# williamyang98/FM-Radio

Hardware: AMD Instinct MI355X
Metric: IQ MSamples/sec demodulated to stereo+RDS per GPU; channels @ real-time (higher is better)
Workload: dtype f32 (tolerance mode: FIR operands split into 2 x bf16 on the matrix cores, 3 products per tap, fp32 accumulate; everything else fp32)

## Files before the change

fm-radio_amd/csrc/fmd_kernels_bp.inc:

```
struct ExtractGeomB {
    static constexpr int TA = 256, WN = 4 * TA + 188, WNP = 1216;
    static constexpr int NBW = (WNP + 8 * (WNP >> 5)) / 2;
    static constexpr int KS = 8;
    static constexpr int EDGE = 124;
    __device__ static __forceinline__ int pad(int i) { return i + 8 * (i >> 5); }
    static_assert(WNP % 32 == 0 && WNP >= 64 * 15 + 32 * KS, "reach of the operands");
    static_assert(WN % 4 == 0 && WN / 4 - 256 <= 64 && WNP / 4 - 256 <= 64, "four quads per lane and one more for lanes 0 .. 47 stage the window");
};
static constexpr int kBpTabU4 = kBpTL * 2 / 16, kBpTabSlotU4 = kBpSlotTabs * kBpTabU4;
static_assert(kBpTL * 2 % 256 == 128 && kBpTL >= kBpPadL + 4 + 32 * ExtractGeomB::KS + 8 && kBpPadL >= 32 + 4 * 14 + 8 && kBpPadL % 8 == 0, "tap table geometry");

__device__ __forceinline__ float oct_sum_f32(float v) {
    {
        const int up = __builtin_amdgcn_update_dpp(0, __float_as_int(v), 0x104, 0xf, 0x5, true);
        v += __int_as_float(__builtin_amdgcn_update_dpp(up, __float_as_int(v), 0x114, 0xf, 0xA, false));
    }
    v += dpp0<0x4E>(v);
    v += dpp0<0xB1>(v);
    return v;
}

template <int SPW>
__global__ __launch_bounds__(256, 4) void k_extract_bp(Dims d, int nt, const float* __restrict__ fo_pl, const float4* __restrict__ pll_poly,
                                                        const uint4* __restrict__ bp_tab, const int2* __restrict__ aud_idx, const uint4* __restrict__ rds_tab,
                                                        const uint4* __restrict__ bp_edge, const float* __restrict__ mixctl, float* __restrict__ state,
                                                        float* __restrict__ audio, float2* __restrict__ rds, float* __restrict__ lmr_est,
                                                        float* __restrict__ lpr_out, float* __restrict__ lmr_out, int keep_taps,
                                                        const float* __restrict__ lmr_est_prev, int field_cur, int field_prev, float* __restrict__ rds_pow) {
    using G = ExtractGeomB;
    constexpr int TA = G::TA;
    __shared__ __attribute__((aligned(256))) uint16_t tabs[(kBpSlotTabs + kBpRdsTabs) * kBpTL];
    __shared__ __attribute__((aligned(16))) uint32_t win[4][2 * G::NBW];
    __shared__ float2 s_old[SPW][SPW == 1 ? 32 : 31];
    __shared__ float off_s[SPW];
    float* wf32 = reinterpret_cast<float*>(win[3]);
    static_assert(sizeof(tabs) + sizeof(win) + sizeof(s_old) + sizeof(off_s) <= 40960, "four workgroups per CU");

    const bool no_edge = (nt & 0x10000) != 0;
    nt &= 0xffff;
    const int tiles = d.n_audio / TA, per_wg = 4 * nt, groups = (tiles + per_wg - 1) / per_wg;
    const int c = SPW * (blockIdx.x / groups), tile_first = (blockIdx.x % groups) * per_wg;
    const bool two = SPW == 2 && c + 1 < d.C;
    const int tid = threadIdx.x;
    __builtin_assume(tid >= 0 && tid < 256);
    const int lane = tid & (kWave - 1), wv = __builtin_amdgcn_readfirstlane(tid >> 6);
    const int n = d.n_fm_out;
    const float* fo_c0 = fo_pl + (size_t)c * (kFoPad + n) + kFoPad;
    const float4* po_c0 = pll_poly + (size_t)c * (1 + n / kSpan) + 1;
    const float off_prev0 = st(state, field_prev, d.C, c), off_prev1 = two ? st(state, field_prev, d.C, c + 1) : 0.0f;
    float off_cur0 = lmr_est_prev ? 0.0f : st(state, field_cur, d.C, c), off_cur1 = (lmr_est_prev || !two) ? 0.0f : st(state, field_cur, d.C, c + 1);
    const bool edge = tile_first == 0 && !no_edge;
#ifdef FMD_X_PROBE
    const bool xp_on = (blockIdx.x % 61) == 0;
    unsigned long long xp_t = __builtin_readcyclecounter();
    const unsigned long long xp_c0 = xp_t, xp_w0 = wall_clock64();
    if (xp_on && threadIdx.x == 0) atomicAdd(&g_x_probe[7], (unsigned long long)nt);
#endif

    float ev[kLmrInlineMax / kWave];
    const bool est_wave = wv == 0 || (wv == 1 && two);
    if (lmr_est_prev && est_wave) {
#pragma unroll
        for (int k = 0; k < kLmrInlineMax / kWave; k++) ev[k] = (lane + kWave * k < d.n_est) ? lmr_est_prev[(size_t)(c + wv) * d.n_est + lane + kWave * k] : 0.0f;
    }
    uint4 em[kBpEdgeU4];
    float4 qe, qe1;
    {
        const int2 slot = aud_idx[c];
        if (edge) {
            if (tid < 48) qe = *reinterpret_cast<const float4*>(fo_c0 - 188 + 4 * tid);
            if (SPW == 2 && two && tid < 48) qe1 = *reinterpret_cast<const float4*>(fo_c0 + (kFoPad + n) - 188 + 4 * tid);
            if (tid < kBpEdgeRows) {
                const uint4* ep = bp_edge + ((size_t)slot.y * kBpEdgeRows + tid) * kBpEdgeU4;
#pragma unroll
                for (int k = 0; k < kBpEdgeU4; k++) em[k] = ep[k];
            }
        }
        constexpr int NU4 = (kBpSlotTabs + kBpRdsTabs) * kBpTabU4;
#pragma unroll
        for (int r = 0; r < (NU4 + 255) / 256; r++) {
            const int j = tid + 256 * r;
            if (j < NU4) {
                const int blk = j / (4 * kBpTabU4), within = j % (4 * kBpTabU4);
                const uint4* src = blk == 0 ? bp_tab + (size_t)slot.x * kBpTabSlotU4 + within
                                 : (blk < 3 ? bp_tab + (size_t)slot.y * kBpTabSlotU4 + blk * 4 * kBpTabU4 + within : rds_tab + (blk - 3) * 4 * kBpTabU4 + within);
                reinterpret_cast<uint4*>(tabs)[j] = *src;
            }
        }
    }
    const int mode0 = (int)mixctl[2 * c], mode1 = two ? (int)mixctl[2 * c + 2] : 0;
    const float kmix0 = mixctl[2 * c + 1], kmix1 = two ? mixctl[2 * c + 3] : 0.0f;
    if (lmr_est_prev && est_wave) {
        float part = 0.0f;
#pragma unroll
        for (int k = 0; k < kLmrInlineMax / kWave; k++) part += ev[k];
        float nxt = fmaf(wave_sum_f32(part) * __builtin_amdgcn_rcpf((float)d.n_est), 0.1f, wv ? off_prev1 : off_prev0);
        const float two_pi = bits_f32(kTwoPiBits);
        nxt = (nxt >= two_pi) ? nxt - two_pi : ((nxt <= -two_pi) ? nxt + two_pi : nxt);
        if (lane == 0) { off_s[wv] = nxt; if (tile_first == 0) st(state, field_cur, d.C, c + wv) = nxt; }
    }
#pragma unroll
    for (int sx = 0; sx < SPW; sx++) {
      if (edge && (sx == 0 || two)) {
        if (sx) __syncthreads();
        if (tid < 48) *reinterpret_cast<float4*>(wf32 + 4 * tid) = sx ? qe1 : qe;
        __syncthreads();
        if (tid < kBpEdgeRows) {
            const float* wp = wf32 + 24 * (tid & 7);
            float ar = 0.0f, ai = 0.0f;
            typedef _Float16 h2_t __attribute__((ext_vector_type(2)));
#pragma unroll
            for (int k = 0; k < kBpEdgeU4; k++) {
                const float4 w4 = *reinterpret_cast<const float4*>(wp + 4 * k);
                const uint32_t ew[4] = {em[k].x, em[k].y, em[k].z, em[k].w};
                const float ws[4] = {w4.x, w4.y, w4.z, w4.w};
#pragma unroll
                for (int u = 0; u < 4; u++) {
                    const h2_t e = __builtin_bit_cast(h2_t, ew[u]);
                    ar = fmaf((float)e[0], ws[u], ar); ai = fmaf((float)e[1], ws[u], ai);
                }
            }
            ar = oct_sum_f32(ar); ai = oct_sum_f32(ai);
            if ((tid & 7) == 0) s_old[sx][tid >> 3] = make_float2(ar, ai);
        }
      }
    }
    __syncthreads();
    if (lmr_est_prev) { off_cur0 = off_s[0]; if (SPW == 2 && two) off_cur1 = off_s[1]; }
    X_STAMP(1);

    uint32_t* fh = win[wv];
    uint32_t* fl = fh + G::NBW;
    float4 qw[5];
    const int tiles_wg = two ? 2 * tiles : tiles;
    auto wload = [&](int tix) {
        const int sx = (SPW == 2 && tix >= tiles) ? 1 : 0, tile = tix - sx * tiles;
        const float* wsrc = fo_c0 + (size_t)sx * (kFoPad + n) + (4 * tile * TA - 188);
#pragma unroll
        for (int r = 0; r < 4; r++) qw[r] = ld_mid(reinterpret_cast<const float4*>(wsrc + 4 * (lane + 64 * r)));
        const int q4 = 256 + lane;
        qw[4] = ld_mid(reinterpret_cast<const float4*>(wsrc + 4 * (q4 < G::WN / 4 ? q4 : G::WN / 4 - 1)));
    };
    if (tile_first + wv < tiles_wg) wload(tile_first + wv);
    for (int it = 0; it < nt; it++) {
        const int tix = tile_first + 4 * it + wv;
        if (tix >= tiles_wg) break;
        const int sx = (SPW == 2 && tix >= tiles) ? 1 : 0, tile = tix - sx * tiles, i0 = tile * TA;
        const int cc = c + sx;
        const float4* po_c = po_c0 + (size_t)sx * (1 + n / kSpan);
        const float off_prev = sx ? off_prev1 : off_prev0, off_cur = sx ? off_cur1 : off_cur0, kmix = sx ? kmix1 : kmix0;
        const int mode = sx ? mode1 : mode0;
        int ln = lane;
        asm volatile("" : "+v"(ln));
        __builtin_assume(ln >= 0 && ln < 64);
        const int lrow = ln & 15, lq = ln >> 4;
        const int m0 = i0 + 16 * lrow + 4 * lq, r0 = (i0 >> 1) + 8 * lrow + 2 * lq;
        const int tc2a = 8 * m0 - 121, tc2r = 16 * r0 - 113;

        {
            auto put = [&](int q, const float4& v) {
                uint32_t h0, l0, h1, l1, h2, l2, h3, l3;
                split_bf16(v.x, h0, l0); split_bf16(v.y, h1, l1); split_bf16(v.z, h2, l2); split_bf16(v.w, h3, l3);
                const int w = G::pad(4 * q) >> 1;
                *reinterpret_cast<uint2*>(fh + w) = make_uint2(pack_hi16(h0, h1), pack_hi16(h2, h3));
                *reinterpret_cast<uint2*>(fl + w) = make_uint2(pack_hi16(l0, l1), pack_hi16(l2, l3));
            };
#pragma unroll
            for (int r = 0; r < 4; r++) put(ln + 64 * r, qw[r]);
            if (ln < G::WNP / 4 - 256) put(256 + ln, (256 + ln >= G::WN / 4) ? make_float4(0.f, 0.f, 0.f, 0.f) : qw[4]);
        }
        const float4 pva = po_c[tc2a >> 8], pvr = po_c[tc2r >> 8];
        asm volatile("s_waitcnt lgkmcnt(0)" ::: "memory");
        __builtin_amdgcn_wave_barrier();
        X_STAMP(0);

        f32x4 acc[4] = {kZero4, kZero4, kZero4, kZero4}, s1 = kZero4;
        {
            const int wb = G::pad(64 * lrow + 8 * lq) >> 1;
            const uint16_t* ta = tabs + (lrow & 1) * kBpTL + kBpPadL + 8 * lq - 4 * (lrow & ~1);
            const uint16_t* t3 = tabs + (12 + (lrow & 1)) * kBpTL + kBpPadL + 8 * lq - 8 * (lrow >> 1);
            auto ld = [](const void* p) { return __builtin_bit_cast(bf16x8, *reinterpret_cast<const uint4*>(p)); };
#pragma unroll
            for (int sK = 0; sK < G::KS; sK++) {
                const bf16x8 bh = ld(fh + wb + 20 * sK), bl = ld(fl + wb + 20 * sK);
                bf16x8 ah[4], al[4];
                ah[0] = ld(ta - 32 + 32 * sK);               al[0] = ld(ta - 32 + 2 * kBpTL + 32 * sK);
                ah[1] = ld(ta + 4 * kBpTL + 32 * sK);        al[1] = ld(ta + 6 * kBpTL + 32 * sK);
                ah[2] = ld(ta + 8 * kBpTL + 32 * sK);        al[2] = ld(ta + 10 * kBpTL + 32 * sK);
                ah[3] = ld(t3 + 32 * sK);                    al[3] = ld(t3 + 2 * kBpTL + 32 * sK);
                const bf16x8 a1 = ld(t3 + 4 * kBpTL + 32 * sK);
#pragma unroll
                for (int f = 0; f < 4; f++) acc[f] = __builtin_amdgcn_mfma_f32_16x16x32_bf16(ah[f], bh, acc[f], 0, 0, 0);
#pragma unroll
                for (int f = 0; f < 4; f++) acc[f] = __builtin_amdgcn_mfma_f32_16x16x32_bf16(al[f], bh, acc[f], 0, 0, 0);
#pragma unroll
                for (int f = 0; f < 4; f++) acc[f] = __builtin_amdgcn_mfma_f32_16x16x32_bf16(ah[f], bl, acc[f], 0, 0, 0);
                s1 = __builtin_amdgcn_mfma_f32_16x16x32_bf16(a1, bh, s1, 0, 0, 0);
#ifndef FMD_BP_SB
#define FMD_BP_SB 1
#endif
                if ((sK % FMD_BP_SB) == FMD_BP_SB - 1) __builtin_amdgcn_sched_barrier(0);
            }
        }
        asm volatile("" ::: "memory");
        X_STAMP(2);
        if (it + 1 < nt && tix + 4 < tiles_wg) wload(tix + 4);

        {
            const float uc0 = 0.5f * (float)(tc2a & 255);
            float dc = 0.0f, ds = 0.0f;
            if (tile == 0) {
                const float dph = off_prev - off_cur;
                dc = fast_cos_turns(dph) - 1.0f; ds = fast_sin_turns(dph);
            }
            float lmr_v[4], lre_v[4], lpr_v[4], au[8];
#pragma unroll
            for (int i = 0; i < 4; i++) {
                const int m = m0 + i;
                const float uc = uc0 + 4.0f * (float)i;
                const float p = fmaf(fmaf(fmaf(pva.w, uc, pva.z), uc, pva.y), uc, pva.x);
                const float nom = (float)((-38 * (4 * (m + 1) - 127)) & 127) * (1.0f / 128.0f);
                float2 sv = make_float2(acc[1][i], acc[2][i]);
                if (tile == 0 && 16 * lrow + 4 * lq + i < 31) {
                    const float2 so = s_old[sx][16 * lrow + 4 * lq + i];
                    sv.x += fmaf(dc, so.x, -(ds * so.y)); sv.y += fmaf(dc, so.y, ds * so.x);
                }
                const float ph = fmaf(2.0f, p, nom) + off_cur;
                const float cs = fast_cos_turns(ph), sn = fast_sin_turns(ph);
                const float lmr_re = fmaf(sv.x, cs, -(sv.y * sn)), lmr = fmaf(sv.x, sn, sv.y * cs);
                const float lpr = acc[0][i];
                float l, r;
                if (mode == FMD_AUDIO_STEREO) { l = fmaf(lmr, kmix, lpr); r = fmaf(-lmr, kmix, lpr); }
                else if (mode == FMD_AUDIO_LMR) { l = lmr; r = lmr; }
                else { l = lpr; r = lpr; }
                au[2 * i] = l + l; au[2 * i + 1] = r + r;
                lmr_v[i] = lmr; lre_v[i] = lmr_re; lpr_v[i] = lpr;
            }
            float4* ap = reinterpret_cast<float4*>(audio + 2 * ((size_t)cc * d.n_audio + m0));
            st_stream(ap, make_float4(au[0], au[1], au[2], au[3])); st_stream(ap + 1, make_float4(au[4], au[5], au[6], au[7]));
            if (keep_taps) {
                *reinterpret_cast<float4*>(lpr_out + (size_t)cc * d.n_audio + m0) = make_float4(lpr_v[0], lpr_v[1], lpr_v[2], lpr_v[3]);
                *reinterpret_cast<float4*>(lmr_out + (size_t)cc * d.n_audio + m0) = make_float4(lmr_v[0], lmr_v[1], lmr_v[2], lmr_v[3]);
            }
            {
                const int k10 = (10 - m0 % 10) % 10;
                if (k10 < 4) {
                    const float a = k10 == 0 ? lmr_v[0] : (k10 == 1 ? lmr_v[1] : (k10 == 2 ? lmr_v[2] : lmr_v[3]));
                    const float b = k10 == 0 ? lre_v[0] : (k10 == 1 ? lre_v[1] : (k10 == 2 ? lre_v[2] : lre_v[3]));
                    const float pe = fast_atan2f(a, b);
                    const float half_pi = bits_f32(kHalfPiBits);
                    lmr_est[(size_t)cc * d.n_est + (m0 + k10) / 10] = (pe > 0.0f) ? (half_pi - pe) : (-half_pi - pe);
                }
            }
            {
                const float ur0 = 0.5f * (float)(tc2r & 255);
                float y[4], pw[2];
#pragma unroll
                for (int j = 0; j < 2; j++) {
                    const int ri = r0 + j;
                    const float ur = ur0 + 8.0f * (float)j;
                    const float pr = fmaf(fmaf(fmaf(pvr.w, ur, pvr.z), ur, pvr.y), ur, pvr.x);
                    const float dpr = fmaf(fmaf(3.0f * pvr.w, ur, 2.0f * pvr.z), ur, pvr.y);
                    const float nomr = (float)((-57 * (8 * (ri + 1) - 127)) & 127) * (1.0f / 128.0f);
                    const float eps = bits_f32(kTwoPiBits) * 3.0f * dpr;
                    const float xr = fmaf(-eps, s1[2 * j + 1], acc[3][2 * j]), xi = fmaf(eps, s1[2 * j], acc[3][2 * j + 1]);
                    const float phr = fmaf(3.0f, pr, nomr);
                    const float cr = fast_cos_turns(phr), sr = fast_sin_turns(phr);
                    y[2 * j] = fmaf(xr, cr, -(xi * sr)); y[2 * j + 1] = fmaf(xr, sr, xi * cr);
                    pw[j] = wave_sum_f32(fmaf(y[2 * j], y[2 * j], y[2 * j + 1] * y[2 * j + 1]));
                }
                *reinterpret_cast<float4*>(rds + (size_t)cc * d.n_rds + r0) = make_float4(y[0], y[1], y[2], y[3]);
                if (ln == 0) *reinterpret_cast<float2*>(rds_pow + ((size_t)cc * tiles + tile) * 2) = make_float2(pw[0], pw[1]);
            }
        }
        X_STAMP(3);
        X_STAMP(4);
    }
#ifdef FMD_X_PROBE
    if (xp_on && (threadIdx.x & 63) == 0 && (threadIdx.x >> 6) == 0) { atomicAdd(&g_x_probe2[7], __builtin_readcyclecounter() - xp_c0); atomicAdd(&g_x_probe2[15], wall_clock64() - xp_w0); }
#endif
}
```

fm-radio_amd/csrc/fmd_tables.cpp:

```cpp
#include "fmd_tables.h"

#include <cmath>
#include <complex>
#include <cstring>
#include <vector>

#include "fmd_design.h"
#include "fmd_math.h"
#include "fmdemod_debug.h"

namespace fmd {

static uint16_t bf16_rne(float x) {
    uint32_t u; std::memcpy(&u, &x, 4);
    u += 0x7fffu + ((u >> 16) & 1u);
    return (uint16_t)(u >> 16);
}
static float bf16_to_f32(uint16_t h) { const uint32_t u = (uint32_t)h << 16; float x; std::memcpy(&x, &u, 4); return x; }
static void toeplitz_image(const float* taps, int n_taps, int stride, int ksteps, uint16_t* img, int shift = 0) {
    for (int sK = 0; sK < ksteps; sK++)
        for (int l = 0; l < 64; l++)
            for (int i = 0; i < 8; i++) {
                const int t = 32 * sK + 8 * (l / 16) + i, idx = t - shift - stride * (l % 16);
                const float v = (idx >= 0 && idx < n_taps) ? taps[idx] : 0.0f;
                const uint16_t hi = bf16_rne(v), lo = bf16_rne(v - bf16_to_f32(hi));
                img[(((size_t)sK * 2 + 0) * 64 + l) * 8 + i] = hi;
                img[(((size_t)sK * 2 + 1) * 64 + l) * 8 + i] = lo;
            }
}

static void bandpass_taps(const float* h, const float* b_hil, int H, float* g_re, float* g_im) {
    double re[kBpTaps] = {0.0}, im[kBpTaps] = {0.0};
    const double two_pi = 6.283185307179586476925;
    for (int tau = 0; tau < 128; tau++) {
        const int k = (H * 19 * tau) % 128;
        const double cr = std::cos(two_pi * k / 128.0), ci = -std::sin(two_pi * k / 128.0), hv = h[tau];
        re[tau + 32] += hv * cr; im[tau + 32] += hv * ci;
        for (int n = 0; n < 65; n++) {
            const double b = b_hil[n];
            if (b == 0.0) continue;
            re[tau + n] += hv * (-ci) * b;
            im[tau + n] += hv * cr * b;
        }
    }
    for (int u = 0; u < kBpTaps; u++) { g_re[u] = (float)re[u]; g_im[u] = (float)im[u]; }
}
static void bp_tap_table(const float* taps, int n_taps, int move, uint16_t* hi, uint16_t* lo) {
    for (int i = 0; i < kBpTL; i++) { hi[i] = 0; if (lo) lo[i] = 0; }
    for (int i = 0; i < n_taps; i++) {
        const uint16_t h = bf16_rne(taps[i]);
        hi[kBpPadL + move + i] = h;
        if (lo) lo[kBpPadL + move + i] = bf16_rne(taps[i] - bf16_to_f32(h));
    }
}
static void bp_family_block(const float* taps, int n_taps, uint16_t* dst) {
    bp_tap_table(taps, n_taps, 0, dst, dst + 2 * kBpTL);
    bp_tap_table(taps, n_taps, 4, dst + kBpTL, dst + 3 * kBpTL);
}
void bp_slot_tap_tables(const float* taps, const float* b_hil, uint16_t* dst) {
    bp_family_block(taps, 128, dst);
    float gr[kBpTaps], gi[kBpTaps];
    bandpass_taps(taps, b_hil, 2, gr, gi);
    bp_family_block(gr, kBpTaps, dst + 4 * kBpTL);
    bp_family_block(gi, kBpTaps, dst + 8 * kBpTL);
}
void bp_rds_tap_tables(const float* b_rds, const float* b_hil, uint16_t* dst) {
    float gr[kBpTaps], gi[kBpTaps], h1[128];
    bandpass_taps(b_rds, b_hil, 3, gr, gi);
    bp_tap_table(gr, kBpTaps, 4, dst, dst + 2 * kBpTL);
    bp_tap_table(gi, kBpTaps, 4, dst + kBpTL, dst + 3 * kBpTL);
    for (int i = 0; i < 128; i++) h1[i] = (float)(((double)i - 63.5) * (double)b_rds[i]);
    bandpass_taps(h1, b_hil, 3, gr, gi);
    bp_tap_table(gr, kBpTaps, 4, dst + 4 * kBpTL, nullptr);
    bp_tap_table(gi, kBpTaps, 4, dst + 5 * kBpTL, nullptr);
}

static uint16_t f32_to_f16_rne(float x) {
    uint32_t u; std::memcpy(&u, &x, 4);
    const uint32_t sign = (u >> 16) & 0x8000u;
    const int e = (int)((u >> 23) & 0xffu) - 127 + 15;
    uint32_t m = u & 0x7fffffu;
    if (e >= 31) return (uint16_t)(sign | 0x7c00u);
    if (e <= 0) {
        if (e < -10) return (uint16_t)sign;
        m |= 0x800000u;
        const int sh = 14 - e;
        const uint32_t r = m >> sh, rem = m & ((1u << sh) - 1u), half = 1u << (sh - 1);
        return (uint16_t)(sign | (r + ((rem > half || (rem == half && (r & 1u))) ? 1u : 0u)));
    }
    const uint32_t r = ((uint32_t)e << 10) | (m >> 13), rem = m & 0x1fffu;
    return (uint16_t)(sign | (r + ((rem > 0x1000u || (rem == 0x1000u && (r & 1u))) ? 1u : 0u)));
}
void bp_edge_matrix(const float* taps, const float* b_hil, uint16_t* dst) {
    constexpr int NM = kBpEdgeRows / 8, NC = kBpEdgeU4 * 4;
    static_assert(8 * NC == kBpTaps, "eight lanes share an output's taps");
    std::memset(dst, 0, sizeof(uint16_t) * kBpEdgeHalves);
    for (int m = 0; m < NM; m++) {
        float ht[128], gr[kBpTaps], gi[kBpTaps];
        for (int i = 0; i < 128; i++) ht[i] = i < 124 - 4 * m ? taps[i] : 0.0f;
        bandpass_taps(ht, b_hil, 2, gr, gi);
        for (int u = 0; u < kBpTaps; u++) {
            const int idx = u - 4 * m;
            if (idx < 0 || idx >= kBpTaps) continue;
            uint16_t* e = dst + (((size_t)m * 8 + u / NC) * NC + u % NC) * 2;
            e[0] = f32_to_f16_rne(gr[idx]); e[1] = f32_to_f16_rne(gi[idx]);
        }
    }
}

void design_pilot_fast(const fmd_coeffs& k, PilotFastTab* t) {
    const double a0 = k.pilot_a[0], a1 = k.pilot_a[1];
    struct M2 { double a, b, c, d; };
    auto mul = [](const M2& x, const M2& y) { return M2{x.a * y.a + x.b * y.c, x.a * y.b + x.b * y.d, x.c * y.a + x.d * y.c, x.c * y.b + x.d * y.d}; };
    const M2 A{a1, a0, 1.0, 0.0};
    M2 P = A;
    for (int i = 0; i < kPilotSeg; i++) { t->h1[i] = (float)P.a; t->h2[i] = (float)P.b; if (i + 1 < kPilotSeg) P = mul(A, P); }
    M2 S = P;
    for (int s = 0; s < 4; s++) { t->m[s][0] = (float)S.a; t->m[s][1] = (float)S.b; t->m[s][2] = (float)S.c; t->m[s][3] = (float)S.d; S = mul(S, S); }
    M2 L{1.0, 0.0, 0.0, 1.0};
    for (int l = 0; l <= 32; l++) { t->mlane[l][0] = (float)L.a; t->mlane[l][1] = (float)L.b; t->mlane[l][2] = (float)L.c; t->mlane[l][3] = (float)L.d; L = mul(P, L); }
    t->k = k.pilot_b[0]; t->a0 = k.pilot_a[0]; t->a1 = k.pilot_a[1];
}

static void span_rows(const fmd_coeffs& k, std::vector<double> (&rows)[kSpanRows]) {
    constexpr int L = kSpan, NV = 5 + L;
    const double b0 = k.pll_lpf_b[0], b1 = k.pll_lpf_b[1], a0 = k.pll_lpf_a[0];
    const float Ts32 = 1.0f / 128000.0f;
    const double Ts = (double)Ts32, ktsi = (double)(0.1f * Ts32), two_pi = 6.283185307179586476925;
    using Vec = std::vector<double>;
    auto unit = [&](int i) { Vec v(NV, 0.0); v[(size_t)i] = 1.0; return v; };
    Vec lpf = unit(0), I = unit(1), e1 = unit(2), e2 = unit(3), dev(NV, 0.0), g0;
    for (int n = 0; n < L; n++) {
        Vec g(NV), e(NV);
        for (int i = 0; i < NV; i++) {
            lpf[i] = b0 * e2[i] + b1 * e1[i] + a0 * lpf[i];
            I[i] += ktsi * e1[i];
            g[i] = -100.0 * (0.01 * lpf[i] + I[i]);
        }
        if (n == 0) g0 = g;
        for (int i = 0; i < NV; i++) dev[i] += Ts * (g[i] - g0[i]);
        dev[4] -= Ts;
        for (int i = 0; i < NV; i++) e[i] = two_pi * dev[i];
        e[5 + n] += two_pi;
        if (n == kSpanN1) rows[2] = dev;
        if (n == kSpanN2) rows[3] = dev;
        if (n == L - 1) { rows[0] = lpf; rows[1] = I; rows[4] = dev; }
        e2 = e1; e1 = e;
    }
}

static void span_cubic_inverse(float (&minv)[3][4]) {
    constexpr int L = kSpan;
    const double x[3] = {(double)kSpanN1, (double)kSpanN2, (double)(L - 1)};
    double A[3][3], inv[3][3];
    for (int i = 0; i < 3; i++) { A[i][0] = x[i]; A[i][1] = x[i] * x[i]; A[i][2] = x[i] * x[i] * x[i]; }
    const double det = A[0][0] * (A[1][1] * A[2][2] - A[1][2] * A[2][1]) - A[0][1] * (A[1][0] * A[2][2] - A[1][2] * A[2][0]) + A[0][2] * (A[1][0] * A[2][1] - A[1][1] * A[2][0]);
    for (int i = 0; i < 3; i++)
        for (int j = 0; j < 3; j++) {
            const int i1 = (i + 1) % 3, i2 = (i + 2) % 3, j1 = (j + 1) % 3, j2 = (j + 2) % 3;
            inv[j][i] = (A[i1][j1] * A[i2][j2] - A[i1][j2] * A[i2][j1]) / det;
        }
    for (int i = 0; i < 3; i++) { for (int j = 0; j < 3; j++) minv[i][j] = (float)inv[i][j]; minv[i][3] = 0.0f; }
}

void design_pll_span(const fmd_coeffs& k, PllSpanTab* t) {
    constexpr int L = kSpan;
    const float Ts32 = 1.0f / 128000.0f;
    const double Ts = (double)Ts32, two_pi = 6.283185307179586476925;
    std::vector<double> rows[kSpanRows];
    span_rows(k, rows);
    std::memset(t, 0, sizeof(*t));
    for (int r = 0; r < kSpanRows; r++) {
        for (int n = 0; n < L; n++) t->w[r][n] = (float)rows[r][(size_t)(5 + n)];
        for (int i = 0; i < 5; i++) t->s[r][i] = (float)rows[r][(size_t)i];
    }
    span_cubic_inverse(t->minv);
    const double w0 = two_pi * 19000.0 / 128000.0;
    double hr = 0.0, hi = 0.0;
    for (int i = 0; i < 65; i++) { hr += k.b_hilbert[i] * std::cos(w0 * i); hi += k.b_hilbert[i] * std::sin(w0 * i); }
    t->quad = (float)(std::sqrt(hr * hr + hi * hi) / (2.0 * std::sin(w0)));
    t->kappa = (float)(-19000.0 * Ts + 19.0 / 128.0);
    for (int i = 0; i < 32; i++) t->hil[i] = k.b_hilbert[2 * i + 1];
}

void design_pll_sparse(const fmd_coeffs& k, PllSparseTab* t) {
    using cd = std::complex<double>;
    constexpr int L = kSpan, D = kSparseDec, KP = kSparsePts;
    const double two_pi = 6.283185307179586476925, w0 = two_pi * 19.0 / 128.0;
    const float Ts32 = 1.0f / 128000.0f;
    std::memset(t, 0, sizeof(*t));
    const double r = std::sqrt(-(double)k.pilot_a[0]), wp = std::acos((double)k.pilot_a[1] / (2.0 * r));
    const cd rho = std::polar(r, wp - w0);
    cd W[2 * D];
    for (int q = -8; q < 24; q++) {
        cd acc = 0.0;
        for (int i = 0; i < D; i++) if (std::abs(q - i) <= 8) acc += std::pow(rho, i);
        W[q + 8] = acc / 17.0;
    }
    cd wcd[2 * D];
    for (int tt = 0; tt < 2 * D; tt++) {
        wcd[tt] = W[(23 - tt) + 8] * std::polar(1.0, -w0 * (double)(tt - 46));
        t->wre[tt] = (float)wcd[tt].real(); t->wim[tt] = (float)wcd[tt].imag();
    }
    const cd rho16 = std::pow(rho, D);
    for (int kk = 0; kk < KP; kk++) {
        const cd ro = std::polar(1.0, -w0 * (double)(D * kk)), ca = std::pow(rho16, kk + 1);
        t->rot[kk][0] = (float)ro.real(); t->rot[kk][1] = (float)ro.imag();
        t->carry[kk][0] = (float)ca.real(); t->carry[kk][1] = (float)ca.imag();
        t->nk1[kk] = (float)(D * kk + 10);
    }
    double nbar = 0.0, s2 = 0.0;
    for (int kk = 0; kk < KP; kk++) nbar += (double)(D * kk + 9) / KP;
    for (int kk = 0; kk < KP; kk++) { const double c = (double)(D * kk + 9) - nbar; t->ck[kk] = (float)c; s2 += c * c; }
    for (int s_ = 0; s_ < 3; s_++) { const cd p = std::pow(rho16, 1 << s_); t->scan[s_][0] = (float)p.real(); t->scan[s_][1] = (float)p.imag(); }
    const cd cA = cd(0.0, -1.0) * ((double)k.pilot_b[0] / std::sin(wp)) * std::polar(1.0, wp);
    double phi0 = std::arg(cA) / two_pi - 19.0 * 33.0 / 128.0;
    phi0 -= std::nearbyint(phi0);
    t->phi0 = (float)phi0; t->inv_s2 = (float)(1.0 / s2); t->nbar = (float)nbar;
    t->kappa = (float)(-19000.0 * (double)Ts32 + 19.0 / 128.0);
    double hr = 0.0, hi = 0.0;
    for (int i = 0; i < 65; i++) { hr += k.b_hilbert[i] * std::cos(w0 * i); hi += k.b_hilbert[i] * std::sin(w0 * i); }
    const double g2 = hr * hr + hi * hi;
    t->pw_scale = (float)(std::norm(cA) * (1.0 + g2) * 0.5 * (double)D);
    cd wdc = 0.0;
    for (int q = 0; q < 2 * D; q++) wdc += W[q];
    const cd kap2 = -std::polar(1.0, -2.0 * wp) / (wdc * (1.0 - std::polar(r, -(wp + w0))));
    t->kap2[0] = (float)kap2.real(); t->kap2[1] = (float)kap2.imag();
    std::vector<double> rows[kSpanRows];
    span_rows(k, rows);
    {
        float mi[3][4];
        span_cubic_inverse(mi);
        const std::vector<double> d1 = rows[2], d2 = rows[3], d3 = rows[4];
        for (int i = 0; i < 3; i++)
            for (size_t j = 0; j < d1.size(); j++) rows[2 + i][j] = (double)mi[i][0] * d1[j] + (double)mi[i][1] * d2[j] + (double)mi[i][2] * d3[j];
    }
    for (int rr = 0; rr < kSpanRows; rr++) {
        double ws = 0.0, wm = 0.0, suf = 0.0;
        for (int n = L - 1; n >= 0; n--) {
            const double w = rows[rr][(size_t)(5 + n)];
            ws += w; wm += w * ((double)n - nbar); suf += w;
            t->sw[rr][n] = (float)suf;
        }
        t->wsum[rr] = (float)ws; t->wmom[rr] = (float)wm;
        for (int i = 0; i < 5; i++) t->s[rr][i] = (float)rows[rr][(size_t)i];
    }
}

void design_wrap_tie(uint32_t* bits2048) {
    std::memset(bits2048, 0, sizeof(uint32_t) * 2048);
    const float pi = fmd::bits_f32(fmd::kPiBits), two_pi = fmd::bits_f32(fmd::kTwoPiBits);
    for (int yr = 0; yr < 256; yr++)
        for (int xr = 0; xr < 256; xr++) {
            const float x = (float)xr - 127.0f, y = (float)yr - 127.0f;
            if (x == 0.0f && y == 0.0f) continue;
            float dl = fmd::fmd_atan2f_full(0.0f - y, 0.0f - x) - fmd::fmd_atan2f_full(y, x);
            if (dl >= pi) dl = dl - two_pi;
            else if (dl <= -pi) dl = dl + two_pi;
            const unsigned key = ((unsigned)yr << 8) | (unsigned)xr;
            if (dl > 0.0f) bits2048[key >> 5] |= 1u << (key & 31u);
        }
}

void design_front_mfma(const fmd_coeffs& k, int m, std::vector<uint16_t>& img) {
    const int ks_pre = m > 1 ? predecim_ksteps(m) : 0;
    img.assign(((size_t)kFrontImgU4 + (size_t)ks_pre * kImgKStepU4) * 8, 0);
    toeplitz_image(k.b_fm_out, 64, 2, 3, img.data());
    toeplitz_image(k.b_hilbert, 65, 1, 3, img.data() + (size_t)kFrontImgU4 / 2 * 8);
    if (m > 1) toeplitz_image(k.b_fm_in, 64, m, ks_pre, img.data() + (size_t)kFrontImgU4 * 8, predecim_shift(m));
}

}

using namespace fmd;

int fmd_design_pll_span(int fs_baseband, float* w, float* s, float* minv, float* misc2) {
    if (!w || !s || !minv || !misc2) return FMD_ERR_ARG;
    if (fs_baseband != 256000 && fs_baseband != 1024000 && fs_baseband != 2048000) return FMD_ERR_ARG;
    fmd_controls def;
    fmd_default_controls(&def);
    fmd_coeffs k{};
    design_all(&k, fs_baseband, &def);
    PllSpanTab t;
    design_pll_span(k, &t);
    std::memcpy(w, t.w, sizeof(t.w)); std::memcpy(s, t.s, sizeof(t.s)); std::memcpy(minv, t.minv, sizeof(t.minv));
    misc2[0] = t.quad; misc2[1] = t.kappa;
    return FMD_OK;
}

int fmd_design_pll_sparse(int fs_baseband, float* taps, float* cplx, float* rows, float* sw, float* misc8) {
    if (!taps || !cplx || !rows || !sw || !misc8) return FMD_ERR_ARG;
    if (fs_baseband != 256000 && fs_baseband != 1024000 && fs_baseband != 2048000) return FMD_ERR_ARG;
    fmd_controls def;
    fmd_default_controls(&def);
    fmd_coeffs k{};
    design_all(&k, fs_baseband, &def);
    PllSparseTab t;
    design_pll_sparse(k, &t);
    std::memcpy(taps, t.wre, sizeof(t.wre)); std::memcpy(taps + 2 * kSparseDec, t.wim, sizeof(t.wim));
    std::memcpy(cplx, t.rot, sizeof(t.rot)); std::memcpy(cplx + 16, t.scan, sizeof(t.scan)); std::memcpy(cplx + 22, t.carry, sizeof(t.carry));
    std::memcpy(rows, t.wsum, sizeof(t.wsum)); std::memcpy(rows + 8, t.wmom, sizeof(t.wmom));
    std::memcpy(sw, t.sw, sizeof(t.sw));
    const float m[8] = {t.phi0, t.inv_s2, t.nbar, t.kappa, t.pw_scale, t.kap2[0], t.kap2[1], 0.f};
    std::memcpy(misc8, m, sizeof(m));
    return FMD_OK;
}

int fmd_design_wrap_tie(uint32_t* bits2048) {
    if (!bits2048) return FMD_ERR_ARG;
    design_wrap_tie(bits2048);
    return FMD_OK;
}

int fmd_design_extract_bp(int fs_baseband, int cutoff_hz, float* g2, float* g3) {
    if (!g2 || !g3) return FMD_ERR_ARG;
    fmd_controls c;
    fmd_default_controls(&c);
    c.lmr_cutoff_hz = cutoff_hz;
    fmd_coeffs k{};
    design_all(&k, fs_baseband, &c);
    bandpass_taps(k.b_lmr, k.b_hilbert, 2, g2, g2 + kBpTaps);
    bandpass_taps(k.b_rds, k.b_hilbert, 3, g3, g3 + kBpTaps);
    return FMD_OK;
}
```

fm-radio_amd/csrc/fmd_tables.h:

```cpp
#pragma once

#include <stddef.h>
#include <stdint.h>
#include <vector>

#include "fmdemod.h"

namespace fmd {

static constexpr int kPilotSeg = 8;
struct PilotFastTab {
    float h1[kPilotSeg], h2[kPilotSeg];
    float m[4][4];
    float mlane[33][4];
    float k, a0, a1;
};

static constexpr int kSpan = 128;
static constexpr int kSpanN1 = 41, kSpanN2 = 84;
static constexpr int kSpanRows = 5;
struct PllSpanTab {
    float w[kSpanRows][kSpan];
    float s[kSpanRows][8];
    float minv[3][4];
    float quad;
    float kappa;
    float pad[2];
    float hil[32];
};
static constexpr int kSparsePts = 8, kSparseDec = kSpan / kSparsePts;
static constexpr float kPllWarmSamples = 8192.0f;
struct PllSparseTab {
    float wre[2 * kSparseDec], wim[2 * kSparseDec];
    float rot[kSparsePts][2];
    float scan[3][2];
    float carry[kSparsePts][2];
    float ck[kSparsePts];
    float nk1[kSparsePts];
    float phi0;
    float inv_s2, nbar, kappa, pw_scale;
    float kap2[2], pad_;
    float wsum[8], wmom[8];
    float s[kSpanRows][8];
    float sw[kSpanRows][kSpan + 4];
    uint32_t wrap_tie[2048];
};
static constexpr int kImgKStepU4 = 2 * 64;
static constexpr int kFrontImgU4 = 2 * 3 * kImgKStepU4;
constexpr int predecim_shift(int m) { return 8 - m; }
constexpr int predecim_ksteps(int m) { return (64 + predecim_shift(m) + 15 * m + 31) / 32; }
static constexpr int kFoPad = 192;

static constexpr int kBpTaps = 192;
static constexpr int kBpPadL = 96, kBpTL = 448;
static constexpr int kBpSlotTabs = 12, kBpRdsTabs = 6;
static constexpr size_t kBpTabSlotU16 = (size_t)kBpSlotTabs * kBpTL, kBpRdsTabU16 = (size_t)kBpRdsTabs * kBpTL;
static constexpr int kBpEdgeRows = 31 * 8, kBpEdgeU4 = 6;
static constexpr size_t kBpEdgeHalves = (size_t)kBpEdgeRows * kBpEdgeU4 * 8;

void design_pilot_fast(const fmd_coeffs& k, PilotFastTab* t);
void design_pll_span(const fmd_coeffs& k, PllSpanTab* t);
void design_pll_sparse(const fmd_coeffs& k, PllSparseTab* t);
void design_wrap_tie(uint32_t* bits2048);
void design_front_mfma(const fmd_coeffs& k, int m, std::vector<uint16_t>& img);
void bp_slot_tap_tables(const float* taps, const float* b_hil, uint16_t* dst);
void bp_rds_tap_tables(const float* b_rds, const float* b_hil, uint16_t* dst);
void bp_edge_matrix(const float* taps, const float* b_hil, uint16_t* dst);

}
```

Baseline: 264,900.

## Give each wave consecutive tiles, slide the LDS window, skip zero-tap L+R MFMAs

Each wave now handles a contiguous run of tiles rather than interleaving with stride 4. That lets it keep the overlapping tail of the previous split-bf16 window in LDS, slide it forward, and convert only the new quads instead of reloading and re-splitting the whole window. The L+R filter family skips the first and last K-steps, whose 128-tap table holds only zeros, removing three MFMAs per skipped step. This trades the prior cross-wave load balancing and coalescing pattern for less global traffic and conversion work, plus an extra LDS copy with an explicit wait.

Measured after the change: 261,100. 0.986x the previous value.

```diff
diff --git a/fm-radio_amd/csrc/fmd_kernels_bp.inc b/fm-radio_amd/csrc/fmd_kernels_bp.inc
--- a/fm-radio_amd/csrc/fmd_kernels_bp.inc
+++ b/fm-radio_amd/csrc/fmd_kernels_bp.inc
@@ -3,10 +3,18 @@
     static constexpr int NBW = (WNP + 8 * (WNP >> 5)) / 2;
     static constexpr int KS = 8;
     static constexpr int EDGE = 124;
+    static constexpr int ROW = 4;
+    static constexpr int LPR_SHIFT = 32;
+    static constexpr int SLIDE_G0 = 4 * TA / 32, SLIDE_GROUPS = (WNP - 4 * TA) / 32, NEW_Q0 = (WN - 4 * TA) / 4;
     __device__ static __forceinline__ int pad(int i) { return i + 8 * (i >> 5); }
+    static constexpr bool lpr_step(int s) { return 32 * s + 31 - LPR_SHIFT >= 0 && 32 * s - LPR_SHIFT - ROW * 15 < kBpLprTaps; }
+    static_assert((4 * TA) % 32 == 0 && SLIDE_G0 + SLIDE_GROUPS == WNP / 32 && 4 * SLIDE_GROUPS * 2 <= 64 && WN / 4 - NEW_Q0 == 256 && WNP / 4 - WN / 4 == 1,
+                  "slide: whole padded groups, a 16-byte move per lane, four new quads per lane, one quad of zeros behind the window");
     static_assert(WNP % 32 == 0 && WNP >= 64 * 15 + 32 * KS, "reach of the operands");
     static_assert(WN % 4 == 0 && WN / 4 - 256 <= 64 && WNP / 4 - 256 <= 64, "four quads per lane and one more for lanes 0 .. 47 stage the window");
 };
+static_assert(!ExtractGeomB::lpr_step(0) && !ExtractGeomB::lpr_step(ExtractGeomB::KS - 1) && ExtractGeomB::lpr_step(1) && ExtractGeomB::lpr_step(ExtractGeomB::KS - 2),
+              "L+R: K-steps 0 and KS - 1 multiply zero taps only (and are left out), the others do not");
 static constexpr int kBpTabU4 = kBpTL * 2 / 16, kBpTabSlotU4 = kBpSlotTabs * kBpTabU4;
 static_assert(kBpTL * 2 % 256 == 128 && kBpTL >= kBpPadL + 4 + 32 * ExtractGeomB::KS + 8 && kBpPadL >= 32 + 4 * 14 + 8 && kBpPadL % 8 == 0, "tap table geometry");
 
@@ -57,6 +65,19 @@
     if (xp_on && threadIdx.x == 0) atomicAdd(&g_x_probe[7], (unsigned long long)nt);
 #endif
 
+    float4 qw[5];
+    const int tiles_wg = two ? 2 * tiles : tiles, tix0 = tile_first + wv * nt;
+    auto wload = [&](int tix, bool slide) {
+        const int sx = (SPW == 2 && tix >= tiles) ? 1 : 0, tile = tix - sx * tiles;
+        const float* wsrc = fo_c0 + (size_t)sx * (kFoPad + n) + (4 * tile * TA - 188) + (slide ? 4 * G::NEW_Q0 : 0);
+#pragma unroll
+        for (int r = 0; r < 4; r++) qw[r] = ld_mid(reinterpret_cast<const float4*>(wsrc + 4 * (lane + 64 * r)));
+        if (!slide) {
+            const int q4 = 256 + lane;
+            qw[4] = ld_mid(reinterpret_cast<const float4*>(wsrc + 4 * (q4 < G::WN / 4 ? q4 : G::WN / 4 - 1)));
+        }
+    };
+
     float ev[kLmrInlineMax / kWave];
     const bool est_wave = wv == 0 || (wv == 1 && two);
     if (lmr_est_prev && est_wave) {
@@ -88,6 +109,7 @@
             }
         }
     }
+    if (tix0 < tiles_wg) wload(tix0, false);
     const int mode0 = (int)mixctl[2 * c], mode1 = two ? (int)mixctl[2 * c + 2] : 0;
     const float kmix0 = mixctl[2 * c + 1], kmix1 = two ? mixctl[2 * c + 3] : 0.0f;
     if (lmr_est_prev && est_wave) {
@@ -131,21 +153,11 @@
 
     uint32_t* fh = win[wv];
     uint32_t* fl = fh + G::NBW;
-    float4 qw[5];
-    const int tiles_wg = two ? 2 * tiles : tiles;
-    auto wload = [&](int tix) {
-        const int sx = (SPW == 2 && tix >= tiles) ? 1 : 0, tile = tix - sx * tiles;
-        const float* wsrc = fo_c0 + (size_t)sx * (kFoPad + n) + (4 * tile * TA - 188);
-#pragma unroll
-        for (int r = 0; r < 4; r++) qw[r] = ld_mid(reinterpret_cast<const float4*>(wsrc + 4 * (lane + 64 * r)));
-        const int q4 = 256 + lane;
-        qw[4] = ld_mid(reinterpret_cast<const float4*>(wsrc + 4 * (q4 < G::WN / 4 ? q4 : G::WN / 4 - 1)));
-    };
-    if (tile_first + wv < tiles_wg) wload(tile_first + wv);
     for (int it = 0; it < nt; it++) {
-        const int tix = tile_first + 4 * it + wv;
+        const int tix = tix0 + it;
         if (tix >= tiles_wg) break;
         const int sx = (SPW == 2 && tix >= tiles) ? 1 : 0, tile = tix - sx * tiles, i0 = tile * TA;
+        const bool slide = it > 0 && tile != 0;
         const int cc = c + sx;
         const float4* po_c = po_c0 + (size_t)sx * (1 + n / kSpan);
         const float off_prev = sx ? off_prev1 : off_prev0, off_cur = sx ? off_cur1 : off_cur0, kmix = sx ? kmix1 : kmix0;
@@ -165,9 +177,20 @@
                 *reinterpret_cast<uint2*>(fh + w) = make_uint2(pack_hi16(h0, h1), pack_hi16(h2, h3));
                 *reinterpret_cast<uint2*>(fl + w) = make_uint2(pack_hi16(l0, l1), pack_hi16(l2, l3));
             };
-#pragma unroll
-            for (int r = 0; r < 4; r++) put(ln + 64 * r, qw[r]);
-            if (ln < G::WNP / 4 - 256) put(256 + ln, (256 + ln >= G::WN / 4) ? make_float4(0.f, 0.f, 0.f, 0.f) : qw[4]);
+            if (slide) {
+                constexpr int U4 = 4 * G::SLIDE_GROUPS;
+                if (ln < 2 * U4) {
+                    uint32_t* half = ln < U4 ? fh : fl;
+                    const int u = ln < U4 ? ln : ln - U4, w = 20 * (u >> 2) + 4 * (u & 3);
+                    const uint4 ov = *reinterpret_cast<const uint4*>(half + 20 * G::SLIDE_G0 + w);
+                    asm volatile("s_waitcnt lgkmcnt(0)" ::: "memory");
+                    *reinterpret_cast<uint4*>(half + w) = ov;
+                }
+            }
+            const int qb = slide ? G::NEW_Q0 : 0;
+#pragma unroll
+            for (int r = 0; r < 4; r++) put(qb + ln + 64 * r, qw[r]);
+            if (!slide && ln < G::WNP / 4 - 256) put(256 + ln, (256 + ln >= G::WN / 4) ? make_float4(0.f, 0.f, 0.f, 0.f) : qw[4]);
         }
         const float4 pva = po_c[tc2a >> 8], pvr = po_c[tc2r >> 8];
         asm volatile("s_waitcnt lgkmcnt(0)" ::: "memory");
@@ -177,24 +200,26 @@
         f32x4 acc[4] = {kZero4, kZero4, kZero4, kZero4}, s1 = kZero4;
         {
             const int wb = G::pad(64 * lrow + 8 * lq) >> 1;
-            const uint16_t* ta = tabs + (lrow & 1) * kBpTL + kBpPadL + 8 * lq - 4 * (lrow & ~1);
+            const uint16_t* ta = tabs + (lrow & 1) * kBpTL + kBpPadL + 8 * lq - G::ROW * (lrow & ~1);
             const uint16_t* t3 = tabs + (12 + (lrow & 1)) * kBpTL + kBpPadL + 8 * lq - 8 * (lrow >> 1);
             auto ld = [](const void* p) { return __builtin_bit_cast(bf16x8, *reinterpret_cast<const uint4*>(p)); };
 #pragma unroll
             for (int sK = 0; sK < G::KS; sK++) {
                 const bf16x8 bh = ld(fh + wb + 20 * sK), bl = ld(fl + wb + 20 * sK);
+                const bool lpr = G::lpr_step(sK);
+                const int f0 = lpr ? 0 : 1;
                 bf16x8 ah[4], al[4];
-                ah[0] = ld(ta - 32 + 32 * sK);               al[0] = ld(ta - 32 + 2 * kBpTL + 32 * sK);
+                if (lpr) { ah[0] = ld(ta - G::LPR_SHIFT + 32 * sK); al[0] = ld(ta - G::LPR_SHIFT + 2 * kBpTL + 32 * sK); }
                 ah[1] = ld(ta + 4 * kBpTL + 32 * sK);        al[1] = ld(ta + 6 * kBpTL + 32 * sK);
                 ah[2] = ld(ta + 8 * kBpTL + 32 * sK);        al[2] = ld(ta + 10 * kBpTL + 32 * sK);
                 ah[3] = ld(t3 + 32 * sK);                    al[3] = ld(t3 + 2 * kBpTL + 32 * sK);
                 const bf16x8 a1 = ld(t3 + 4 * kBpTL + 32 * sK);
 #pragma unroll
-                for (int f = 0; f < 4; f++) acc[f] = __builtin_amdgcn_mfma_f32_16x16x32_bf16(ah[f], bh, acc[f], 0, 0, 0);
-#pragma unroll
-                for (int f = 0; f < 4; f++) acc[f] = __builtin_amdgcn_mfma_f32_16x16x32_bf16(al[f], bh, acc[f], 0, 0, 0);
-#pragma unroll
-                for (int f = 0; f < 4; f++) acc[f] = __builtin_amdgcn_mfma_f32_16x16x32_bf16(ah[f], bl, acc[f], 0, 0, 0);
+                for (int f = f0; f < 4; f++) acc[f] = __builtin_amdgcn_mfma_f32_16x16x32_bf16(ah[f], bh, acc[f], 0, 0, 0);
+#pragma unroll
+                for (int f = f0; f < 4; f++) acc[f] = __builtin_amdgcn_mfma_f32_16x16x32_bf16(al[f], bh, acc[f], 0, 0, 0);
+#pragma unroll
+                for (int f = f0; f < 4; f++) acc[f] = __builtin_amdgcn_mfma_f32_16x16x32_bf16(ah[f], bl, acc[f], 0, 0, 0);
                 s1 = __builtin_amdgcn_mfma_f32_16x16x32_bf16(a1, bh, s1, 0, 0, 0);
 #ifndef FMD_BP_SB
 #define FMD_BP_SB 1
@@ -204,7 +229,7 @@
         }
         asm volatile("" ::: "memory");
         X_STAMP(2);
-        if (it + 1 < nt && tix + 4 < tiles_wg) wload(tix + 4);
+        if (it + 1 < nt && tix + 1 < tiles_wg) wload(tix + 1, !(SPW == 2 && tix + 1 == tiles));
 
         {
             const float uc0 = 0.5f * (float)(tc2a & 255);
diff --git a/fm-radio_amd/csrc/fmd_tables.cpp b/fm-radio_amd/csrc/fmd_tables.cpp
--- a/fm-radio_amd/csrc/fmd_tables.cpp
+++ b/fm-radio_amd/csrc/fmd_tables.cpp
@@ -58,7 +58,7 @@
     bp_tap_table(taps, n_taps, 4, dst + kBpTL, dst + 3 * kBpTL);
 }
 void bp_slot_tap_tables(const float* taps, const float* b_hil, uint16_t* dst) {
-    bp_family_block(taps, 128, dst);
+    bp_family_block(taps, kBpLprTaps, dst);
     float gr[kBpTaps], gi[kBpTaps];
     bandpass_taps(taps, b_hil, 2, gr, gi);
     bp_family_block(gr, kBpTaps, dst + 4 * kBpTL);
diff --git a/fm-radio_amd/csrc/fmd_tables.h b/fm-radio_amd/csrc/fmd_tables.h
--- a/fm-radio_amd/csrc/fmd_tables.h
+++ b/fm-radio_amd/csrc/fmd_tables.h
@@ -52,6 +52,7 @@
 static constexpr int kFoPad = 192;
 
 static constexpr int kBpTaps = 192;
+static constexpr int kBpLprTaps = 128;
 static constexpr int kBpPadL = 96, kBpTL = 448;
 static constexpr int kBpSlotTabs = 12, kBpRdsTabs = 6;
 static constexpr size_t kBpTabSlotU16 = (size_t)kBpSlotTabs * kBpTL, kBpRdsTabU16 = (size_t)kBpRdsTabs * kBpTL;
```
